# danini/multi-h

Measured on AMD Instinct MI355X. Metric: scored homography hypotheses/sec (50k pts x 100k models), higher is better.
Workload: dtype f64

## Files before the change

multi-h_amd/csrc/expand.hip:

```cpp

#include "mh_kernels.hpp"

#include <algorithm>
#include <atomic>
#include <chrono>

namespace mh {

enum { C_TLAST = 0,
       C_PEND = 1,
       C_ERROR = 2,
       C_ACCEPTED = 3,
       C_EXCESS_NODES = 4,
       C_ARRIVE = 5,
       C_TICKET = 6,
       C_FLOW_MOVES = 7,
       C_CORE = 8,
       C_MOVES_SOLVED = 16, C_CORE_MAX = 17, C_MOVES_RUN = 18, C_XCD_USED = 19,
       C_TOOK_N = 20,
       C_XCD = 64, C_LINE = 32, C_TOP = C_XCD + 8 * C_LINE,
       C_SUBTICKET = C_TOP + C_LINE, SUBTICKETS = 16,
       C_COUNT = EXPAND_FLAG_WORDS };
static_assert(C_SUBTICKET + SUBTICKETS * C_LINE <= C_COUNT, "control block too small");
constexpr int STRIPES = 64, STRIPE_LL = 16;
enum { A_DELTA_S = 64, A_ENERGY_S = A_DELTA_S + STRIPES * STRIPE_LL, A_EXCESS_S = A_ENERGY_S + STRIPES * STRIPE_LL,
       A_TOTAL = A_EXCESS_S + STRIPES * STRIPE_LL };
static_assert(A_TOTAL <= EXPAND_ACC_WORDS, "accumulator block too small");
enum { A_DELTA = 0, A_ENERGY = 1, A_EXCESS_SUM = 2, A_CORE_SUM = 3, A_OUTER = 4, A_RELAX = 5, A_PUSH = 6,
       A_BARRIERS = 7, A_TICKS = 8, A_T_BAR = 9, A_T_RELAX = 10, A_T_PUSH = 11, A_T_TAIL = 12, A_TAIL_ROUNDS = 13, A_MAX_WAIT = 14, A_COUNT = 16  };
enum { ERR_OVERFLOW = 1, ERR_BARRIER_TIMEOUT = 2, ERR_NO_CONVERGENCE = 3 };

struct MoveCtx {
    int* cap; int* sent; int* excess; int* sink_cap; int* height; int* decided; unsigned char* took; int* core;
    int* took_list;
    int* flags; long long* acc;
    int* saved_flow; int* saved_sink; int* trace; int* detail;
    int alpha, t, warm;
};
struct MoveBatch { MoveCtx c[EXPAND_MAX_CTX]; int count; };
enum { B_TLAST0 = 0,
       B_SEQ = 1,
       B_TICKET = 2,
       B_BAD = 8,
       B_WORDS = 8 + EXPAND_MAX_CTX };
static_assert(EXPAND_MAX_CTX <= 32, "one bit per move of a batch");
enum { HB_FIRST_INVALID = 0, HB_TLAST = 1, HB_ERROR = 2, HB_ACCEPTED_HERE = 3, HB_DIRTY = 4, HB_SEQ = 5, HB_WORDS = 8 };

#define LD(p) __hip_atomic_load((p), __ATOMIC_RELAXED, __HIP_MEMORY_SCOPE_AGENT)
#define ST(p, v) __hip_atomic_store((p), (v), __ATOMIC_RELAXED, __HIP_MEMORY_SCOPE_AGENT)

__device__ __forceinline__ bool move_is_skipped(const int* flags, int t, int L)
{
    return flags[C_ERROR] != 0 || (t >= L && flags[C_TLAST] <= t - L);
}

__global__ void k_ctl_init(MoveBatch b)
{
    int* flags = b.c[blockIdx.x].flags;
    long long* acc = b.c[blockIdx.x].acc;
    for (int t = threadIdx.x; t < C_COUNT; t += blockDim.x) flags[t] = (t == C_TLAST || t == C_PEND) ? -1 : 0;
    for (int t = threadIdx.x; t < A_TOTAL; t += blockDim.x) acc[t] = 0;
}

__global__ void __launch_bounds__(256)
k_init_labeling(const int* __restrict__ cost, int L, int n, const int* __restrict__ init,
                int* __restrict__ label, int* __restrict__ cur_cost)
{
    const int i = blockIdx.x * 256 + threadIdx.x;
    if (i >= n) return;
    const int l = init ? init[i] : 0;
    label[i] = l;
    cur_cost[i] = cost[(size_t)i * L + l];
}

__global__ void __launch_bounds__(256)
k_argmin_labels(const int* __restrict__ cost, int L, int n, int* __restrict__ label,
                long long* __restrict__ acc)
{
    const int i = blockIdx.x * 256 + threadIdx.x;
    long long mine = 0;
    if (i < n) {
        int best = 0, bc = cost[(size_t)i * L];
        for (int l = 1; l < L; ++l) {
            const int c = cost[(size_t)i * L + l];
            if (c < bc) { bc = c; best = l; }
        }
        label[i] = best;
        mine = bc;
    }
    __shared__ long long s[256];
    s[threadIdx.x] = mine;
    __syncthreads();
    for (int st = 128; st >= 1; st >>= 1) {
        if ((int)threadIdx.x < st) s[threadIdx.x] += s[threadIdx.x + st];
        __syncthreads();
    }
    if (threadIdx.x == 0)
        atomicAdd((unsigned long long*)&acc[A_ENERGY_S + (blockIdx.x % STRIPES) * STRIPE_LL], (unsigned long long)s[0]);
}

constexpr int LPN = 16;
constexpr int SITES_PER_BLOCK = 256 / LPN;

template <int CTRL>
__device__ __forceinline__ int dpp_mov(int v) { return __builtin_amdgcn_update_dpp(0, v, CTRL, 0xf, 0xf, true); }
template <int CTRL>
__device__ __forceinline__ long long dpp_mov64(long long v)
{
    const int lo = dpp_mov<CTRL>((int)(unsigned)((unsigned long long)v & 0xffffffffull)), hi = dpp_mov<CTRL>((int)(v >> 32));
    return (long long)(((unsigned long long)(unsigned)hi << 32) | (unsigned)lo);
}
constexpr int DPP_XOR1 = 0xB1, DPP_XOR2 = 0x4E, DPP_HALF_MIRROR = 0x141, DPP_MIRROR = 0x140;
template <int W>
__device__ __forceinline__ int row_min(int v)
{
    static_assert(W == 8 || W == 16, "a DPP row");
    int o = dpp_mov<DPP_XOR1>(v); v = o < v ? o : v;
    o = dpp_mov<DPP_XOR2>(v); v = o < v ? o : v;
    o = dpp_mov<DPP_HALF_MIRROR>(v); v = o < v ? o : v;
    if (W == 16) { o = dpp_mov<DPP_MIRROR>(v); v = o < v ? o : v; }
    return v;
}
template <int W>
__device__ __forceinline__ long long row_min64(long long v)
{
    static_assert(W == 8 || W == 16, "a DPP row");
    long long o = dpp_mov64<DPP_XOR1>(v); v = o < v ? o : v;
    o = dpp_mov64<DPP_XOR2>(v); v = o < v ? o : v;
    o = dpp_mov64<DPP_HALF_MIRROR>(v); v = o < v ? o : v;
    if (W == 16) { o = dpp_mov64<DPP_MIRROR>(v); v = o < v ? o : v; }
    return v;
}
template <int W>
__device__ __forceinline__ long long row_sum64(long long v)
{
    static_assert(W == 8 || W == 16, "a DPP row");
    v += dpp_mov64<DPP_XOR1>(v);
    v += dpp_mov64<DPP_XOR2>(v);
    v += dpp_mov64<DPP_HALF_MIRROR>(v);
    if (W == 16) v += dpp_mov64<DPP_MIRROR>(v);
    return v;
}
template <int W>
__device__ __forceinline__ int row_sum(int v)
{
    static_assert(W == 8 || W == 16, "a DPP row");
    v += dpp_mov<DPP_XOR1>(v);
    v += dpp_mov<DPP_XOR2>(v);
    v += dpp_mov<DPP_HALF_MIRROR>(v);
    if (W == 16) v += dpp_mov<DPP_MIRROR>(v);
    return v;
}

template <typename F>
__device__ __forceinline__ void for_flagged(unsigned long long mask, F body)
{
    const int grp = (int)(threadIdx.x & 63) / LPN;
    while (mask) {
        int b[4];
#pragma unroll
        for (int q = 0; q < 4; ++q) {
            b[q] = mask ? (int)__builtin_ctzll(mask) : -1;
            if (mask) mask &= mask - 1;
        }
        const int m = grp == 0 ? b[0] : grp == 1 ? b[1] : grp == 2 ? b[2] : b[3];
        body(m);
    }
}
constexpr int SPW = 16;
constexpr int SPW_MAX = 64;
constexpr int SITES_PER_WBLOCK_MAX = 4 * SPW_MAX;

__global__ void __launch_bounds__(256)
k_move_setup(Graph g, const int* __restrict__ cost, int L, int potts, int reduce_on,
             int* label, int* __restrict__ cur_cost, MoveBatch b, int spw)
{
    const MoveCtx& c = b.c[blockIdx.y];
    const int alpha = c.alpha, t = c.t;
    const unsigned char* __restrict__ took = c.took;
    int* __restrict__ cap = c.cap;
    int* __restrict__ excess = c.excess;
    int* __restrict__ sink_cap = c.sink_cap;
    int* __restrict__ decided = c.decided;
    int* __restrict__ flags = c.flags;
    long long* __restrict__ acc = c.acc;
    const int lane = threadIdx.x & 63;
    const int sub = threadIdx.x % LPN;
    const int s0 = (blockIdx.x * 4 + (int)(threadIdx.x >> 6)) * spw;
    const int i = s0 + lane;
    const bool in = lane < spw && i < g.n;
    const int pa = flags[C_PEND];
    int li = 0, cc = 0;
    if (in) {
        li = label[i];
        cc = cur_cost[i];
        if (pa >= 0 && took[i]) {
            li = pa;
            cc = cost[(size_t)i * L + pa];
            label[i] = pa; cur_cost[i] = cc;
        }
    }
    if (__shfl(move_is_skipped(flags, t, L) ? 1 : 0, 0)) return;
    long long K = 0;
    bool walk = false;
    if (in) {
        if (li == alpha) decided[i] = 3;
        else {
            K = cost[(size_t)i * L + alpha];
            if (reduce_on && K - cc > 2ll * potts * g.wsum[i]) decided[i] = 2;
            else walk = true;
        }
    }
    for_flagged(__ballot(walk), [&](int m) {
        const int mm = m < 0 ? 0 : m;
        const int li_m = __shfl(li, mm), cc_m = __shfl(cc, mm);
        const long long K_m = __shfl(K, mm);
        if (m < 0) return;
        const int im = s0 + m;
        const int k0 = g.rowptr[im], k1 = g.rowptr[im + 1];
        long long S = 0, out = 0, inn = 0;
        for (int k = k0 + sub; k < k1; k += LPN) {
            const int j = g.col[k];
            const long long wk64 = (long long)g.w[k] * potts;
            if (wk64 > 0x7fffffffll) atomicExch(&flags[C_ERROR], ERR_OVERFLOW);
            const int wk = wk64 > 0x7fffffffll ? 0x7fffffff : (int)wk64;
            int lj = label[j];
            if (pa >= 0 && took[j]) lj = pa;
            if (lj == alpha) { S += wk; cap[k] = 0; cap[g.rev[k]] = 0; }
            else if (j < im) { if (li_m != lj) S += wk; cap[k] = wk; out += wk; if (li_m == lj) inn += wk; }
            else { const int c = (li_m == lj) ? wk : 0; cap[k] = c; out += c; inn += wk; }
        }
        S = row_sum64<LPN>(S) + cc_m;
        out = row_sum64<LPN>(out);
        inn = row_sum64<LPN>(inn);
        if (sub != 0) return;
        const long long tr = S - K_m;
        if (tr > 0x7fffffffll || -tr > 0x7fffffffll) atomicExch(&flags[C_ERROR], ERR_OVERFLOW);
        const int ex = tr > 0 ? (int)tr : 0;
        excess[im] = ex;
        sink_cap[im] = tr < 0 ? (int)(-tr) : 0;
        int verdict = 0;
        if (reduce_on) {
            if (tr > out) verdict = 1;
            else if (-tr > inn) verdict = 2;
        }
        decided[im] = verdict;
        if (ex > 0) atomicAdd((unsigned long long*)&acc[A_EXCESS_S + (blockIdx.x % STRIPES) * STRIPE_LL], (unsigned long long)ex);
    });
}

template <bool COMPACT>
__global__ void __launch_bounds__(256)
k_reduce(Graph g, int L, MoveBatch b, int ROUNDS, int housekeep, int spw)
{
    const MoveCtx& c = b.c[blockIdx.y];
    const int t = c.t;
    int* cap = c.cap;
    int* excess = c.excess;
    int* sink_cap = c.sink_cap;
    int* decided = c.decided;
    int* __restrict__ flags = c.flags;
    long long* __restrict__ acc = c.acc;
    int* __restrict__ core = c.core;
    const int lane = threadIdx.x & 63;
    const int sub = threadIdx.x % LPN;
    const int slot = (blockIdx.x * 4 + (int)(threadIdx.x >> 6)) * spw + lane;
    const int u = (lane < spw && slot < g.n) ? (COMPACT ? g.order[slot] : slot) : -1;
    __shared__ int s_skip;
    __shared__ int s_cnt, s_base;
    __shared__ int s_list[SITES_PER_WBLOCK_MAX];
    if (threadIdx.x == 0) { s_skip = move_is_skipped(flags, t, L) ? 1 : 0; s_cnt = 0; }
    __syncthreads();
    const bool skipped = s_skip != 0;
    if (housekeep && blockIdx.x == 0 && threadIdx.x == 0) {
// ... 649 lines not shown
    __syncthreads();
    int rounds = 0;
    for (;;) {
        if (threadIdx.x == 0) s_changed = 0;
        __syncthreads();
        for (int i = threadIdx.x; i < g.n; i += 1024) {
            int c = comp[i];
            if (c < 0) continue;
            int m = c;
            for (int k = g.rowptr[i]; k < g.rowptr[i + 1]; ++k) { const int cj = comp[g.col[k]]; if (cj >= 0 && cj < m) m = cj; }
            if (m < c) { atomicMin(&comp[i], m); atomicMin(&comp[c], m); s_changed = 1; }
        }
        __syncthreads();
        for (int i = threadIdx.x; i < g.n; i += 1024) {
            int c = comp[i];
            if (c < 0) continue;
            while (comp[c] < c) c = comp[c];
            comp[i] = c;
        }
        __syncthreads();
        ++rounds;
        if (!s_changed || rounds > 4096) break;
        __syncthreads();
    }
    for (int i = threadIdx.x; i < g.n; i += 1024) if (comp[i] >= 0) { atomicAdd(&csize[comp[i]], 1); atomicAdd(&s_acc[0], 1); }
    __syncthreads();
    for (int i = threadIdx.x; i < g.n; i += 1024) {
        const int sz = csize[i];
        if (sz <= 0) continue;
        atomicAdd(&s_acc[1], 1);
        const int old = atomicMax(&s_acc[2], sz);
        atomicMax(&s_acc[3], old < sz ? old : sz);
        if (sz <= 64) { atomicAdd(&s_acc[4], sz); atomicAdd(&s_acc[9], 1); }
        if (sz <= 256) { atomicAdd(&s_acc[5], sz); atomicAdd(&s_acc[10], 1); }
        if (sz <= 1024) { atomicAdd(&s_acc[6], sz); atomicAdd(&s_acc[11], 1); }
        if (sz <= 2048) { atomicAdd(&s_acc[7], sz); atomicAdd(&s_acc[12], 1); }
        if (sz <= 8192) { atomicAdd(&s_acc[8], sz); atomicAdd(&s_acc[13], 1); }
    }
    __syncthreads();
    if (threadIdx.x < 16) out[threadIdx.x] = threadIdx.x == 14 ? rounds : s_acc[threadIdx.x];
}

__global__ void __launch_bounds__(SOLVE_THREADS)
k_solve(Graph g, int L, MoveBatch b, int mslots, SolveParams sp)
{
    const MoveCtx& c = b.c[blockIdx.y];
    const int t = c.t, warm = c.warm;
    int* cap = c.cap;
    int* sent = c.sent;
    int* excess = c.excess;
    int* sink_cap = c.sink_cap;
    int* height = c.height;
    int* decided = c.decided;
    const int* __restrict__ core = c.core;
    int* flags = c.flags;
    long long* acc = c.acc;
    int* __restrict__ trace = c.trace;
    int* __restrict__ detail = c.detail;
    int* __restrict__ saved_flow = c.saved_flow;
    int* __restrict__ saved_sink = c.saved_sink;
    extern __shared__ int s_priv[];
    __shared__ int s_red[8];
    __shared__ int s_skip;
    if (threadIdx.x == 0) s_skip = move_is_skipped(flags, t, L) ? 1 : 0;
    __syncthreads();
    if (s_skip) return;
    if (g.n >= H_MASK) { if (threadIdx.x == 0) atomicExch(&flags[C_ERROR], ERR_OVERFLOW); return; }
    int pre[EXPAND_CORE_SHARDS + 1];
    pre[0] = 0;
#pragma unroll
    for (int s = 0; s < EXPAND_CORE_SHARDS; ++s) pre[s + 1] = pre[s] + flags[C_CORE + s];
    const int K = pre[EXPAND_CORE_SHARDS];
    if (K == 0) return;
    int P = (K + SOLVE_ROWS - 1) / SOLVE_ROWS;
    if (P > (int)gridDim.x) P = (int)gridDim.x;
    if ((int)blockIdx.x >= P) return;
    if (K <= P * SOLVE_ROWS) solve_body<false>(g, t, cap, sent, excess, sink_cap, height, decided, core, flags, acc, trace, detail,
                                                saved_flow, saved_sink, warm, mslots, sp, s_priv, s_red, pre, K, P);
    else solve_body<true>(g, t, cap, sent, excess, sink_cap, height, decided, core, flags, acc, trace, detail,
                          saved_flow, saved_sink, warm, mslots, sp, s_priv, s_red, pre, K, P);
}

__global__ void __launch_bounds__(256)
k_delta(Graph g, const int* __restrict__ cost, int L, int potts,
        const int* __restrict__ label, const int* __restrict__ cur_cost, MoveBatch b, int spw)
{
    const MoveCtx& c = b.c[blockIdx.y];
    const int alpha = c.alpha, t = c.t;
    const int* __restrict__ decided = c.decided;
    unsigned char* __restrict__ took = c.took;
    int* __restrict__ flags = c.flags;
    long long* acc = c.acc;
    __shared__ long long s[256];
    __shared__ int s_last;
    if (threadIdx.x == 0) s_last = move_is_skipped(flags, t, L) ? 1 : 0;
    __syncthreads();
    if (s_last) return;
    const int lane = threadIdx.x & 63;
    const int sub = threadIdx.x % LPN;
    const int s0 = (blockIdx.x * 4 + (int)(threadIdx.x >> 6)) * spw;
    const int i = s0 + lane;
    long long mine = 0;
    int oi = 0;
    bool ti = false;
    if (lane < spw && i < g.n) {
        oi = label[i];
        ti = decided[i] == 1;
        took[i] = ti ? 1 : 0;
        if (ti) mine += (long long)cost[(size_t)i * L + alpha] - cur_cost[i];
    }
    if (c.took_list) {
        const unsigned long long tb = __ballot(ti);
        if (tb) {
            int base = 0;
            if (lane == 0) base = atomicAdd(&flags[C_TOOK_N], (int)__popcll(tb));
            base = __shfl(base, 0);
            if (ti) c.took_list[base + (int)__popcll(tb & ((1ull << lane) - 1ull))] = i;
        }
    }
    for_flagged(__ballot(ti), [&](int m) {
        const int oi_m = __shfl(oi, m < 0 ? 0 : m);
        if (m < 0) return;
        const int im = s0 + m;
        for (int k = g.rowptr[im] + sub; k < g.rowptr[im + 1]; k += LPN) {
            const int j = g.col[k];
            const bool tj = decided[j] == 1;
            if (tj && j > im) continue;
            const int oj = label[j];
            const int nj = tj ? alpha : oj;
            const int dn = (alpha != nj) - (oi_m != oj);
            mine += (long long)dn * g.w[k] * potts;
        }
    });
    s[threadIdx.x] = mine;
    __syncthreads();
    for (int st = 128; st >= 1; st >>= 1) {
        if ((int)threadIdx.x < st) s[threadIdx.x] += s[threadIdx.x + st];
        __syncthreads();
    }
    if (threadIdx.x == 0) {
        if (s[0] != 0) atomicAdd((unsigned long long*)&acc[A_DELTA_S + (blockIdx.x % STRIPES) * STRIPE_LL], (unsigned long long)s[0]);
        asm volatile("s_waitcnt vmcnt(0)" ::: "memory");
        const int st = (int)(blockIdx.x % SUBTICKETS);
        const int members = ((int)gridDim.x - st + SUBTICKETS - 1) / SUBTICKETS;
        int last = 0;
        if (atomicAdd(&flags[C_SUBTICKET + st * C_LINE], 1) == members - 1) {
            const int used = (int)gridDim.x < SUBTICKETS ? (int)gridDim.x : SUBTICKETS;
            last = atomicAdd(&flags[C_TICKET], 1) == used - 1;
        }
        s_last = last;
    }
    __syncthreads();
    if (s_last && threadIdx.x < 64) {
        long long d = (int)threadIdx.x < STRIPES ? LD(&acc[A_DELTA_S + threadIdx.x * STRIPE_LL]) : 0ll;
#pragma unroll
        for (int m = 32; m >= 1; m >>= 1) d += __shfl_xor(d, m, 64);
        if (threadIdx.x == 0 && d < 0) {
            flags[C_TLAST] = t;
            flags[C_PEND] = alpha;
            flags[C_ACCEPTED] += 1;
        }
        if (threadIdx.x == 0) {
            flags[C_MOVES_RUN] += 1;
            for (int s = 0; s < EXPAND_CORE_SHARDS; ++s) flags[C_CORE + s] = 0;
            for (int s = C_XCD; s < C_TOP + C_LINE; ++s) flags[s] = 0;
            flags[C_ARRIVE] = 0;
        }
    }
}

__global__ void __launch_bounds__(256)
k_apply_pending(int n, const int* __restrict__ cost, int L, int* __restrict__ label,
                int* __restrict__ cur_cost, const unsigned char* __restrict__ took,
                const int* __restrict__ flags, int )
{
    const int pa = flags[C_PEND];
    if (pa < 0) return;
    const int i = blockIdx.x * 256 + threadIdx.x;
    if (i < n && took[i]) {
        label[i] = pa;
        cur_cost[i] = cost[(size_t)i * L + pa];
    }
}



__global__ void k_batch_prep(MoveBatch b, int* __restrict__ bctl)
{
    int* G = b.c[0].flags;
    const int k = threadIdx.x;
    if (k == 0) { bctl[B_TLAST0] = G[C_TLAST]; G[C_PEND] = -1; }
    if (k < EXPAND_MAX_CTX) bctl[B_BAD + k] = 0;
    if (k >= 1 && k < b.count) {
        int* f = b.c[k].flags;
        f[C_TLAST] = G[C_TLAST];
        f[C_PEND] = -1;
        f[C_ERROR] = G[C_ERROR];
    }
}

__device__ __forceinline__ bool batch_move_skipped(const MoveCtx& c, int tlast0, int L)
{
    return c.flags[C_ERROR] != 0 || (c.t >= L && tlast0 <= c.t - L);
}

__global__ void __launch_bounds__(256)
k_batch_check(Graph g, const int* __restrict__ cost, int L, int potts, const int* __restrict__ label, const int* __restrict__ cur_cost,
              MoveBatch b, int* __restrict__ bctl)
{
    const int j = blockIdx.y;
    if (j + 1 >= b.count) return;
    const MoveCtx& cj = b.c[j];
    const int tlast0 = bctl[B_TLAST0];
    if (batch_move_skipped(cj, tlast0, L) || cj.flags[C_PEND] < 0) return;
    const int nt = cj.flags[C_TOOK_N];
    const int sub = threadIdx.x % LPN;
    const int alpha_j = cj.alpha, later = b.count - 1 - j;
    unsigned bad = 0;
    for (int idx = blockIdx.x * SITES_PER_BLOCK + (int)threadIdx.x / LPN; idx < nt; idx += gridDim.x * SITES_PER_BLOCK) {
        const int p = cj.took_list[idx];
        const int k0 = g.rowptr[p], k1 = g.rowptr[p + 1];
        for (int a = k0 + sub - (sub == 0 ? 1 : 0); a < k1; a = (a < k0 ? k0 : a + LPN)) {
            const int s_ = a < k0 ? p : g.col[a];
            const long long W = (long long)potts * g.wsum[s_];
            const int lb = label[s_];
            const long long Dl = cur_cost[s_];
            const int* row = cost + (size_t)s_ * L + (alpha_j + 1);
            const long long Dj = a < k0 ? (long long)cost[(size_t)s_ * L + alpha_j] : 0;
            for (int q = 0; q < later; ++q) {
                const long long Db = row[q];
                bool ok = lb == alpha_j + 1 + q || Db - Dl > W;
                if (ok && a < k0) ok = Db - Dj > W;
                if (!ok) bad |= 1u << (j + 1 + q);
            }
        }
    }
#pragma unroll
    for (int m = 32; m >= 1; m >>= 1) bad |= (unsigned)__shfl_xor((int)bad, m, 64);
    if ((threadIdx.x & 63) == 0 && bad) atomicOr((unsigned*)&bctl[B_BAD + j], bad);
}

struct CtxFlags { int* p[EXPAND_MAX_CTX]; };
__global__ void __launch_bounds__(256)
k_batch_commit(const int* __restrict__ cost, int L, int* __restrict__ label, int* __restrict__ cur_cost, MoveBatch b,
               int* __restrict__ bctl, int* __restrict__ h_batch, CtxFlags all_flags, int n_ctx_all)
{
    __shared__ int s_first, s_err, s_last_t, s_n_acc;
    __shared__ unsigned s_acc;
    __shared__ int s_ek[EXPAND_MAX_CTX], s_pend[EXPAND_MAX_CTX], s_nt[EXPAND_MAX_CTX];
    __shared__ unsigned s_bad[EXPAND_MAX_CTX];
    __shared__ int s_g[5];
    if ((int)threadIdx.x < b.count) {
        const int* f = b.c[threadIdx.x].flags;
        s_ek[threadIdx.x] = f[C_ERROR];
        s_pend[threadIdx.x] = f[C_PEND];
        s_nt[threadIdx.x] = f[C_TOOK_N];
        s_bad[threadIdx.x] = (unsigned)bctl[B_BAD + threadIdx.x];
    } else if (threadIdx.x >= 64 && threadIdx.x < 69) {
        const int q = threadIdx.x - 64;
        const int* G = b.c[0].flags;
        s_g[q] = q == 0 ? bctl[B_TLAST0] : q == 1 ? G[C_ERROR] : q == 2 ? G[C_TLAST] : q == 3 ? G[C_ACCEPTED] : bctl[B_SEQ];
    }
    __syncthreads();
    if (threadIdx.x == 0) {
        const int tlast0 = s_g[0];
        unsigned accepted = 0;
        int first_invalid = b.count, err = 0, last_t = -1, n_acc = 0;
        for (int k = 0; k < b.count; ++k) {
            const MoveCtx& c = b.c[k];
            const int ek = s_ek[k];
            const bool skipped = ek != 0 || (c.t >= L && tlast0 <= c.t - L);
            bool valid = true;
            if (accepted) {
                if (skipped) valid = false;
                else
                    for (int j = 0; j < k; ++j)
                        if ((accepted >> j & 1u) && (s_bad[j] >> k & 1u)) valid = false;
            }
            if (!valid) { first_invalid = k; break; }
            if (ek) err = ek;
            if (!skipped && s_pend[k] >= 0) { accepted |= 1u << k; last_t = c.t; ++n_acc; }
        }
        s_first = first_invalid; s_err = err; s_acc = accepted; s_last_t = last_t; s_n_acc = n_acc;
    }
    __syncthreads();
    const unsigned accepted = s_acc;
    for (int k = 0; k < b.count; ++k) {
        if (!(accepted >> k & 1u)) continue;
        const MoveCtx& c = b.c[k];
        const int nt = s_nt[k], a = c.alpha;
        for (int i = blockIdx.x * 256 + threadIdx.x; i < nt; i += gridDim.x * 256) {
            const int p = c.took_list[i];
            label[p] = a;
            cur_cost[p] = cost[(size_t)p * L + a];
        }
    }
    __shared__ int s_is_last;
    __syncthreads();
    if (threadIdx.x == 0) {
        __threadfence();
        s_is_last = atomicAdd(&bctl[B_TICKET], 1) == (int)gridDim.x - 1;
    }
    __syncthreads();
    if (s_is_last && threadIdx.x == 0) {
        bctl[B_TICKET] = 0;
        int* G = b.c[0].flags;
        const int g_err = s_g[1] ? s_g[1] : s_err;
        const int g_tlast = s_last_t > s_g[2] ? s_last_t : s_g[2];
        const int seq = s_g[4] + 1;
        if (g_err != s_g[1]) G[C_ERROR] = g_err;
        if (g_tlast != s_g[2]) G[C_TLAST] = g_tlast;
        G[C_ACCEPTED] = s_g[3] + s_n_acc - (int)(accepted & 1u);
        bctl[B_SEQ] = seq;
        h_batch[HB_FIRST_INVALID] = s_first;
        h_batch[HB_TLAST] = g_tlast;
        h_batch[HB_ERROR] = g_err;
        h_batch[HB_ACCEPTED_HERE] = s_n_acc;
        h_batch[HB_DIRTY] = 0;
        __threadfence_system();
        __hip_atomic_store(&h_batch[HB_SEQ], seq, __ATOMIC_RELEASE, __HIP_MEMORY_SCOPE_SYSTEM);
        bctl[B_TLAST0] = g_tlast;
        G[C_PEND] = -1;
        for (int k = 0; k < EXPAND_MAX_CTX; ++k) bctl[B_BAD + k] = 0;
        for (int k = 1; k < n_ctx_all; ++k) {
            int* f = all_flags.p[k];
            f[C_TLAST] = g_tlast;
            f[C_PEND] = -1;
            f[C_ERROR] = g_err;
        }
    }
}

__global__ void k_stats_merge(MoveBatch b)
{
    const int t = threadIdx.x;
    int* G = b.c[0].flags;
    long long* A = b.c[0].acc;
    const int fw[5] = { C_FLOW_MOVES, C_MOVES_SOLVED, C_MOVES_RUN, C_CORE_MAX, C_XCD_USED };
    if (t < 5) {
        const int w = fw[t];
        int v = G[w];
        for (int k = 1; k < b.count; ++k) {
            int* f = b.c[k].flags;
            if (t < 3) v += f[w]; else if (f[w] > v) v = f[w];
            f[w] = 0;
        }
        G[w] = v;
    } else if (t >= 8 && t - 8 + A_CORE_SUM < A_COUNT) {
        const int w = t - 8 + A_CORE_SUM;
        long long v = A[w];
        for (int k = 1; k < b.count; ++k) {
            long long* a = b.c[k].acc;
            if (w == A_MAX_WAIT) { if (a[w] > v) v = a[w]; } else v += a[w];
            a[w] = 0;
        }
        A[w] = v;
    }
}

__global__ void __launch_bounds__(256)
k_energy(Graph g, int potts, const int* __restrict__ label, const int* __restrict__ cur_cost,
         int* __restrict__ flags, long long* __restrict__ acc)
{
    if (blockIdx.x == 0 && threadIdx.x == 0) flags[C_PEND] = -1;
    const int i = blockIdx.x * SITES_PER_BLOCK + threadIdx.x / LPN;
    const int sub = threadIdx.x % LPN;
    long long mine = 0;
    if (i < g.n) {
        if (sub == 0) mine = cur_cost[i];
        const int li = label[i];
        for (int k = g.rowptr[i] + sub; k < g.rowptr[i + 1]; k += LPN) {
            const int j = g.col[k];
            if (j < i && label[j] != li) mine += (long long)g.w[k] * potts;
        }
    }
    __shared__ long long s[256];
    s[threadIdx.x] = mine;
    __syncthreads();
    for (int st = 128; st >= 1; st >>= 1) {
        if ((int)threadIdx.x < st) s[threadIdx.x] += s[threadIdx.x + st];
        __syncthreads();
    }
    if (threadIdx.x == 0)
        atomicAdd((unsigned long long*)&acc[A_ENERGY_S + (blockIdx.x % STRIPES) * STRIPE_LL], (unsigned long long)s[0]);
}

hipError_t launch_init_labeling(const int* cost, int L, int n, const int* init, int* label,
                                int* cur_cost, hipStream_t s)
{
    hipLaunchKernelGGL(k_init_labeling, dim3((n + 255) / 256), dim3(256), 0, s, cost, L, n, init,
                       label, cur_cost);
    return hipGetLastError();
}

hipError_t launch_argmin_labels(const int* cost, int L, int n, int* label, long long* acc,
                                hipStream_t s)
{
    hipLaunchKernelGGL(k_argmin_labels, dim3((n + 255) / 256), dim3(256), 0, s, cost, L, n, label,
                       acc);
    return hipGetLastError();
}

#define RET_IF(x) do { hipError_t e_ = (x); if (e_ != hipSuccess) return e_; } while (0)

__global__ void k_publish(const int* __restrict__ flags, long long* __restrict__ acc,
                          int* __restrict__ h_flags, long long* __restrict__ h_acc)
{
    const int t = threadIdx.x;
    if (t < EXPAND_HOST_WORDS) h_flags[t] = flags[t];
    long long en = t < STRIPES ? acc[A_ENERGY_S + t * STRIPE_LL] : 0ll;
    if (t < STRIPES) acc[A_ENERGY_S + t * STRIPE_LL] = 0;
#pragma unroll
    for (int m = 32; m >= 1; m >>= 1) en += __shfl_xor(en, m, 64);
    if (t < A_COUNT) h_acc[t] = t == A_ENERGY ? en : acc[t];
}

static hipError_t fetch(ExpandWork& w, ExpandStats& st, hipStream_t s)
{
    ++st.host_syncs;
    ++st.launches;
    hipLaunchKernelGGL(k_publish, dim3(1), dim3(64), 0, s, w.flags, w.acc, w.h_flags_dev, w.h_acc_dev);
    RET_IF(hipGetLastError());
    return hipStreamSynchronize(s);
}

hipError_t solver_blocks_per_cu(int* blocks)
{
    return hipOccupancyMaxActiveBlocksPerMultiprocessor(blocks, (const void*)k_solve, SOLVE_THREADS, sizeof(int) * F_FIELDS * SOLVE_ROWS);
}

hipError_t run_expansion(const Graph& g, const int* cost, int L, int potts, ExpandWork& w,
                         int max_cycles, ExpandStats* st, hipStream_t s)
{
    const dim3 grid1((g.n + 255) / 256), blk(256);
    const dim3 grid((g.n + SITES_PER_BLOCK - 1) / SITES_PER_BLOCK);
    auto spw_for = [&](int count) {
        if (w.batch_spw == 16 || w.batch_spw == 32 || w.batch_spw == 64) return w.batch_spw;
        const long long site_moves = (long long)count * g.n;
        return site_moves > (1ll << 19) ? 64 : site_moves > (1ll << 18) ? 32 : 16;
    };
    ExpandStats stats = {};
    const int n_ctx = std::max(1, std::min(w.n_ctx, EXPAND_MAX_CTX));
    MoveBatch all{};
    all.count = n_ctx;
    for (int k = 0; k < n_ctx; ++k) {
        MoveCtx& c = all.c[k];
        if (k == 0) { c.cap = w.cap; c.sent = w.sent; c.excess = w.excess; c.sink_cap = w.sink_cap; c.height = w.height; c.decided = w.decided;
                      c.took = w.took; c.core = w.core; c.flags = w.flags; c.acc = w.acc; c.took_list = w.took_list0; }
        else { const ExpandWork::Ctx& x = w.ctx[k - 1];
               c.cap = x.cap; c.sent = x.sent; c.excess = x.excess; c.sink_cap = x.sink_cap; c.height = x.height; c.decided = x.decided;
               c.took = x.took; c.core = x.core; c.flags = x.flags; c.acc = x.acc; c.took_list = x.took_list; }
    }
    hipLaunchKernelGGL(k_ctl_init, dim3(n_ctx), dim3(64), 0, s, all);
    RET_IF(hipGetLastError());
    ++stats.launches;
    auto finish_cycle = [&]() -> hipError_t {
        if (n_ctx > 1) { hipLaunchKernelGGL(k_stats_merge, dim3(1), dim3(64), 0, s, all); ++stats.launches; }
        return fetch(w, stats, s);
    };

    if (g.nnz == 0) {
        RET_IF(launch_argmin_labels(cost, L, g.n, w.label, w.acc, s));
        RET_IF(fetch(w, stats, s));
        stats.energy = w.h_acc[A_ENERGY];
        if (st) *st = stats;
        return hipSuccess;
    }

    long long energy = 0, old_energy = 0;
    hipLaunchKernelGGL(k_energy, grid, blk, 0, s, g, potts, w.label, w.cur_cost, w.flags, w.acc);
    RET_IF(fetch(w, stats, s));
    stats.launches += 1;
    energy = w.h_acc[A_ENERGY];
    if (energy > 0x7fffffffll) {
        stats.energy = -ERR_OVERFLOW;
        if (st) *st = stats;
        return hipErrorInvalidValue;
    }

    SolveParams sp{ w.reduce_rounds, w.relax_rounds, w.push_cycles, w.push_phases, w.push_mult > 0 ? w.push_mult : 1, 1 << 20, w.cascade_iters,
                    w.barrier_timeout_ticks > 0 ? (unsigned long long)w.barrier_timeout_ticks : 300000000ull,
                    w.barrier_first_timeout_ticks > 0 ? (unsigned long long)w.barrier_first_timeout_ticks : 300000000ull };
    int solve_grid = w.solve_grid > 0 ? w.solve_grid : 128;
    const int mslots = std::max(1, (g.n + solve_grid * SOLVE_ROWS - 1) / (solve_grid * SOLVE_ROWS));
    const size_t solve_lds = sizeof(int) * F_FIELDS * (size_t)mslots * SOLVE_ROWS;
    if (solve_lds > 128 * 1024) return hipErrorOutOfMemory;
    if (solve_lds > 48 * 1024)
        RET_IF(hipFuncSetAttribute((const void*)k_solve, hipFuncAttributeMaxDynamicSharedMemorySize, (int)solve_lds));

    CtxFlags all_flags{};
    for (int k = 0; k < n_ctx; ++k) all_flags.p[k] = all.c[k].flags;
    bool prepared = false;
    int group = 0;
    int injected_ctx = -1;
    auto enqueue_moves = [&](int alpha0, int t0, int count, int cycle) -> hipError_t {
        MoveBatch b = all;
        b.count = count;
        for (int k = 0; k < count; ++k) {
            MoveCtx& c = b.c[k];
            c.alpha = alpha0 + k;
            c.t = t0 + k;
            c.trace = (w.trace && c.t < w.trace_moves) ? w.trace : nullptr;
            c.detail = (w.trace && c.t == w.detail_move) ? w.trace + 8 * (size_t)w.trace_moves : nullptr;
            c.saved_flow = w.saved_flow ? w.saved_flow + (size_t)c.alpha * g.nnz : nullptr;
            c.saved_sink = w.saved_flow ? w.saved_sink + (size_t)c.alpha * g.n : nullptr;
            c.warm = (w.saved_flow && cycle > 1) ? 1 : 0;
            if (count == 1) c.took_list = nullptr;
        }
        const int spw = count > 1 ? spw_for(count) : SPW;
        const int spw_d = count > 1 ? SPW_MAX : SPW;
        const dim3 grid_w((unsigned)((g.n + 4 * spw - 1) / (4 * spw)), (unsigned)count);
        const dim3 grid_d((unsigned)((g.n + 4 * spw_d - 1) / (4 * spw_d)), (unsigned)count);
        if (count > 1 && !prepared) { hipLaunchKernelGGL(k_batch_prep, dim3(1), dim3(64), 0, s, b, w.bctl); ++stats.launches; }
        prepared = count > 1;
        hipLaunchKernelGGL(k_move_setup, grid_w, blk, 0, s, g, cost, L, potts, w.reduce_rounds > 0 ? 1 : 0, w.label, w.cur_cost, b, spw);
        if (w.reduce_launches > 1)
            hipLaunchKernelGGL(HIP_KERNEL_NAME(k_reduce<false>), grid_w, blk, 0, s, g, L, b, w.reduce_rounds, 1, spw);
        hipLaunchKernelGGL(HIP_KERNEL_NAME(k_reduce<true>), grid_w, blk, 0, s, g, L, b, w.reduce_rounds, w.reduce_launches > 1 ? 0 : 1, spw);
        if (count == 1 && w.comp_out && t0 < w.comp_moves)
            hipLaunchKernelGGL(k_core_components, dim3(1), dim3(1024), 0, s, g, L, t0, w.decided, w.flags, w.comp_scratch,
                               w.comp_scratch + g.n, w.comp_out + 16 * (size_t)t0);
        hipLaunchKernelGGL(k_solve, dim3((unsigned)solve_grid, (unsigned)count), dim3(SOLVE_THREADS), solve_lds, s, g, L, b, mslots, sp);
        injected_ctx = -1;
        if (++group == w.inject_group && w.inject_ctx < count) {
            RET_IF(hipMemsetD32Async((hipDeviceptr_t)(b.c[w.inject_ctx].flags + C_ERROR), ERR_NO_CONVERGENCE, 1, s));
            injected_ctx = w.inject_ctx;
        }
        hipLaunchKernelGGL(k_delta, grid_d, blk, 0, s, g, cost, L, potts, w.label, w.cur_cost, b, spw_d);
        if (count > 1) {
            hipLaunchKernelGGL(k_batch_check, dim3(32, (unsigned)count), blk, 0, s, g, cost, L, potts, w.label, w.cur_cost, b, w.bctl);
            hipLaunchKernelGGL(k_batch_commit, dim3(32), blk, 0, s, cost, L, w.label, w.cur_cost, b, w.bctl, w.h_batch_dev, all_flags, n_ctx);
            stats.launches += 2;
        }
        stats.launches += w.reduce_launches > 1 ? 5 : 4;
        if (w.reduce_rounds > 0) stats.reduce_launches += w.reduce_launches > 1 ? 2 : 1;
        return hipGetLastError();
    };

    const bool can_batch = n_ctx > 1 && w.bctl && w.h_batch && L >= 2 && !w.comp_out;
    bool batching = can_batch && L >= w.batch_min_labels;
    if (can_batch) {
        RET_IF(hipMemsetAsync(w.bctl, 0, sizeof(int) * B_WORDS, s));
        w.h_batch[HB_SEQ] = 0;
    }
    int host_tlast = -1;
    bool host_fresh = true;
    int bsize = n_ctx;
    int batch_seq = 0;
    int t = 0;
    for (int cycle = 1; cycle <= max_cycles; ++cycle) {
        old_energy = energy;
        int alpha = 0;
        if (can_batch && cycle >= 2) batching = true;
        while (alpha < L) {
            if (host_fresh && t >= L && host_tlast <= t - L) {
                const int rest = L - alpha;
                stats.moves += rest; stats.host_skipped += rest;
                alpha += rest; t += rest;
                break;
            }
            int B = std::min(bsize, L - alpha);
            if (host_fresh && t + B > host_tlast + L && host_tlast + L > t && t >= L) B = host_tlast + L - t;
            if (!batching || B < 2) {
                RET_IF(enqueue_moves(alpha, t, 1, cycle));
                ++stats.moves; ++stats.solo_moves;
                ++alpha; ++t;
                host_fresh = false;
                continue;
            }
            if (!host_fresh) {
                hipLaunchKernelGGL(k_apply_pending, grid1, blk, 0, s, g.n, cost, L, w.label, w.cur_cost, w.took, w.flags, 1);
                ++stats.launches;
            }
            RET_IF(enqueue_moves(alpha, t, B, cycle));
            ++stats.batches;
            ++stats.host_syncs;
            ++batch_seq;
            {
                volatile int* seq_word = w.h_batch + HB_SEQ;
                const auto t_poll = std::chrono::steady_clock::now();
                bool seen = false;
                for (int spin = 0;; ++spin) {
                    if (*seq_word == batch_seq) { seen = true; break; }
                    if ((spin & 255) == 255 && std::chrono::steady_clock::now() - t_poll > std::chrono::milliseconds(2)) break;
                }
                if (seen) std::atomic_thread_fence(std::memory_order_acquire);
                else RET_IF(hipStreamSynchronize(s));
                if (w.h_batch[HB_SEQ] != batch_seq) return hipErrorUnknown;
            }
            if (w.h_batch[HB_ERROR]) break;
            const int j = w.h_batch[HB_FIRST_INVALID];
            if (injected_ctx >= j) ++stats.injected_discarded;
            host_tlast = w.h_batch[HB_TLAST];
            host_fresh = true;
            stats.moves += j; stats.batch_committed += j;
            alpha += j; t += j;
            if (j < B) {
                ++stats.batch_invalid;
                if (2 * j < B) bsize = std::max(2, bsize / 2);
            } else if (B == bsize) bsize = std::min(n_ctx, 2 * bsize);
        }
        hipLaunchKernelGGL(k_apply_pending, grid1, blk, 0, s, g.n, cost, L, w.label, w.cur_cost, w.took, w.flags, 0);
        hipLaunchKernelGGL(k_energy, grid, blk, 0, s, g, potts, w.label, w.cur_cost, w.flags, w.acc);
        stats.launches += 2;
        RET_IF(finish_cycle());
        stats.cycles = cycle;
        if (w.h_flags[C_ERROR]) {
            stats.energy = -(long long)w.h_flags[C_ERROR];
            if (st) *st = stats;
            return w.h_flags[C_ERROR] == ERR_OVERFLOW ? hipErrorInvalidValue : hipErrorLaunchTimeOut;
        }
        host_tlast = w.h_flags[C_TLAST];
        host_fresh = true;
        energy = w.h_acc[A_ENERGY];
        if (energy == old_energy) break;
    }
    stats.energy = energy;
    stats.accepted = w.h_flags[C_ACCEPTED];
    stats.flow_moves = w.h_flags[C_FLOW_MOVES];
    stats.moves_solved = w.h_flags[C_MOVES_SOLVED];
    stats.moves_run = w.h_flags[C_MOVES_RUN];
    stats.core_sites = w.h_acc[A_CORE_SUM];
    stats.core_max = w.h_flags[C_CORE_MAX];
    stats.outer_iterations = w.h_acc[A_OUTER];
    stats.relax_intervals = w.h_acc[A_RELAX];
// ... 15 lines not shown
```

Measured before the change: 13.41 million.

## Fuse delta, batch check and commit into one move-tail kernel

Merges the separate k_delta, k_batch_check and k_batch_commit kernels (and removes k_batch_prep) into a single k_move_tail kernel. It computes the batch-conflict bits inline while walking each taken site's neighbourhood, then elects a last block via tickets to commit accepted moves and reset per-context flags. bctl initialisation moves into k_ctl_init. The aim is to cut per-batch kernel launches and the redundant second pass over took_list and neighbours, at the price of the commit running serially in one block and more complex ticket synchronisation.

```diff
diff --git a/multi-h_amd/csrc/expand.hip b/multi-h_amd/csrc/expand.hip
--- a/multi-h_amd/csrc/expand.hip
+++ b/multi-h_amd/csrc/expand.hip
@@ -54,10 +54,12 @@
     return flags[C_ERROR] != 0 || (t >= L && flags[C_TLAST] <= t - L);
 }
 
-__global__ void k_ctl_init(MoveBatch b)
+__global__ void k_ctl_init(MoveBatch b, int* __restrict__ bctl)
 {
     int* flags = b.c[blockIdx.x].flags;
     long long* acc = b.c[blockIdx.x].acc;
+    if (blockIdx.x == 0 && bctl)
+        for (int t = threadIdx.x; t < B_WORDS; t += blockDim.x) bctl[t] = t == B_TLAST0 ? -1 : 0;
     for (int t = threadIdx.x; t < C_COUNT; t += blockDim.x) flags[t] = (t == C_TLAST || t == C_PEND) ? -1 : 0;
     for (int t = threadIdx.x; t < A_TOTAL; t += blockDim.x) acc[t] = 0;
 }
@@ -189,7 +191,7 @@
     const int s0 = (blockIdx.x * 4 + (int)(threadIdx.x >> 6)) * spw;
     const int i = s0 + lane;
     const bool in = lane < spw && i < g.n;
-    const int pa = flags[C_PEND];
+    const int pa = b.count > 1 ? -1 : flags[C_PEND];
     int li = 0, cc = 0;
     if (in) {
         li = label[i];
@@ -1005,64 +1007,109 @@
 }
 
 __global__ void __launch_bounds__(256)
-k_delta(Graph g, const int* __restrict__ cost, int L, int potts,
-        const int* __restrict__ label, const int* __restrict__ cur_cost, MoveBatch b, int spw)
-{
-    const MoveCtx& c = b.c[blockIdx.y];
+k_apply_pending(int n, const int* __restrict__ cost, int L, int* __restrict__ label,
+                int* __restrict__ cur_cost, const unsigned char* __restrict__ took,
+                const int* __restrict__ flags, int )
+{
+    const int pa = flags[C_PEND];
+    if (pa < 0) return;
+    const int i = blockIdx.x * 256 + threadIdx.x;
+    if (i < n && took[i]) {
+        label[i] = pa;
+        cur_cost[i] = cost[(size_t)i * L + pa];
+    }
+}
+
+
+
+struct CtxFlags { int* p[EXPAND_MAX_CTX]; };
+__global__ void __launch_bounds__(256)
+k_move_tail(Graph g, const int* __restrict__ cost, int L, int potts, int* label, int* cur_cost, MoveBatch b, int spw,
+            int* bctl, int* h_batch, CtxFlags all_flags, int n_ctx_all)
+{
+    const int y = blockIdx.y;
+    const MoveCtx& c = b.c[y];
     const int alpha = c.alpha, t = c.t;
     const int* __restrict__ decided = c.decided;
     unsigned char* __restrict__ took = c.took;
-    int* __restrict__ flags = c.flags;
+    int* flags = c.flags;
     long long* acc = c.acc;
     __shared__ long long s[256];
-    __shared__ int s_last;
-    if (threadIdx.x == 0) s_last = move_is_skipped(flags, t, L) ? 1 : 0;
-    __syncthreads();
-    if (s_last) return;
-    const int lane = threadIdx.x & 63;
-    const int sub = threadIdx.x % LPN;
-    const int s0 = (blockIdx.x * 4 + (int)(threadIdx.x >> 6)) * spw;
-    const int i = s0 + lane;
-    long long mine = 0;
-    int oi = 0;
-    bool ti = false;
-    if (lane < spw && i < g.n) {
-        oi = label[i];
-        ti = decided[i] == 1;
-        took[i] = ti ? 1 : 0;
-        if (ti) mine += (long long)cost[(size_t)i * L + alpha] - cur_cost[i];
-    }
-    if (c.took_list) {
-        const unsigned long long tb = __ballot(ti);
-        if (tb) {
-            int base = 0;
-            if (lane == 0) base = atomicAdd(&flags[C_TOOK_N], (int)__popcll(tb));
-            base = __shfl(base, 0);
-            if (ti) c.took_list[base + (int)__popcll(tb & ((1ull << lane) - 1ull))] = i;
-        }
-    }
-    for_flagged(__ballot(ti), [&](int m) {
-        const int oi_m = __shfl(oi, m < 0 ? 0 : m);
-        if (m < 0) return;
-        const int im = s0 + m;
-        for (int k = g.rowptr[im] + sub; k < g.rowptr[im + 1]; k += LPN) {
-            const int j = g.col[k];
-            const bool tj = decided[j] == 1;
-            if (tj && j > im) continue;
-            const int oj = label[j];
-            const int nj = tj ? alpha : oj;
-            const int dn = (alpha != nj) - (oi_m != oj);
-            mine += (long long)dn * g.w[k] * potts;
-        }
-    });
-    s[threadIdx.x] = mine;
-    __syncthreads();
-    for (int st = 128; st >= 1; st >>= 1) {
-        if ((int)threadIdx.x < st) s[threadIdx.x] += s[threadIdx.x + st];
+    __shared__ int s_flag;
+    if (threadIdx.x == 0) s_flag = move_is_skipped(flags, t, L) ? 1 : 0;
+    __syncthreads();
+    const bool skipped = s_flag != 0;
+    __syncthreads();
+    if (!skipped) {
+        const int lane = threadIdx.x & 63;
+        const int sub = threadIdx.x % LPN;
+        const int s0 = (blockIdx.x * 4 + (int)(threadIdx.x >> 6)) * spw;
+        const int i = s0 + lane;
+        const int later = b.count - 1 - y;
+        long long mine = 0;
+        unsigned bad = 0;
+        int oi = 0;
+        bool ti = false;
+        if (lane < spw && i < g.n) {
+            oi = label[i];
+            ti = decided[i] == 1;
+            took[i] = ti ? 1 : 0;
+            if (ti) mine += (long long)cost[(size_t)i * L + alpha] - cur_cost[i];
+        }
+        if (c.took_list) {
+            const unsigned long long tb = __ballot(ti);
+            if (tb) {
+                int base = 0;
+                if (lane == 0) base = atomicAdd(&flags[C_TOOK_N], (int)__popcll(tb));
+                base = __shfl(base, 0);
+                if (ti) ST(&c.took_list[base + (int)__popcll(tb & ((1ull << lane) - 1ull))], i);
+            }
+        }
+        for_flagged(__ballot(ti), [&](int m) {
+            const int oi_m = __shfl(oi, m < 0 ? 0 : m);
+            if (m < 0) return;
+            const int im = s0 + m;
+            const int k0 = g.rowptr[im], k1 = g.rowptr[im + 1];
+            for (int k = k0 + sub; k < k1; k += LPN) {
+                const int j = g.col[k];
+                const bool tj = decided[j] == 1;
+                if (tj && j > im) continue;
+                const int oj = label[j];
+                const int nj = tj ? alpha : oj;
+                const int dn = (alpha != nj) - (oi_m != oj);
+                mine += (long long)dn * g.w[k] * potts;
+            }
+            if (later <= 0) return;
+            for (int a = k0 + sub - (sub == 0 ? 1 : 0); a < k1; a = (a < k0 ? k0 : a + LPN)) {
+                const int s_ = a < k0 ? im : g.col[a];
+                const long long W = (long long)potts * g.wsum[s_];
+                const int lb = label[s_];
+                const long long Dl = cur_cost[s_];
+                const int* row = cost + (size_t)s_ * L + (alpha + 1);
+                const long long Dj = a < k0 ? (long long)cost[(size_t)s_ * L + alpha] : 0;
+                for (int q = 0; q < later; ++q) {
+                    const long long Db = row[q];
+                    bool ok = lb == alpha + 1 + q || Db - Dl > W;
+                    if (ok && a < k0) ok = Db - Dj > W;
+                    if (!ok) bad |= 1u << (y + 1 + q);
+                }
+            }
+        });
+        if (later > 0) {
+#pragma unroll
+            for (int m = 32; m >= 1; m >>= 1) bad |= (unsigned)__shfl_xor((int)bad, m, 64);
+            if (lane == 0 && bad) atomicOr((unsigned*)&bctl[B_BAD + y], bad);
+        }
+        asm volatile("s_waitcnt vmcnt(0)" ::: "memory");
+        s[threadIdx.x] = mine;
         __syncthreads();
+        for (int st = 128; st >= 1; st >>= 1) {
+            if ((int)threadIdx.x < st) s[threadIdx.x] += s[threadIdx.x + st];
+            __syncthreads();
+        }
     }
     if (threadIdx.x == 0) {
-        if (s[0] != 0) atomicAdd((unsigned long long*)&acc[A_DELTA_S + (blockIdx.x % STRIPES) * STRIPE_LL], (unsigned long long)s[0]);
+        if (!skipped && s[0] != 0) atomicAdd((unsigned long long*)&acc[A_DELTA_S + (blockIdx.x % STRIPES) * STRIPE_LL], (unsigned long long)s[0]);
         asm volatile("s_waitcnt vmcnt(0)" ::: "memory");
         const int st = (int)(blockIdx.x % SUBTICKETS);
         const int members = ((int)gridDim.x - st + SUBTICKETS - 1) / SUBTICKETS;
@@ -1071,118 +1118,62 @@
             const int used = (int)gridDim.x < SUBTICKETS ? (int)gridDim.x : SUBTICKETS;
             last = atomicAdd(&flags[C_TICKET], 1) == used - 1;
         }
-        s_last = last;
-    }
-    __syncthreads();
-    if (s_last && threadIdx.x < 64) {
+        s_flag = last;
+    }
+    __syncthreads();
+    if (!s_flag) return;
+
+    if (!skipped && threadIdx.x < 64) {
         long long d = (int)threadIdx.x < STRIPES ? LD(&acc[A_DELTA_S + threadIdx.x * STRIPE_LL]) : 0ll;
 #pragma unroll
         for (int m = 32; m >= 1; m >>= 1) d += __shfl_xor(d, m, 64);
-        if (threadIdx.x == 0 && d < 0) {
-            flags[C_TLAST] = t;
-            flags[C_PEND] = alpha;
-            flags[C_ACCEPTED] += 1;
-        }
         if (threadIdx.x == 0) {
+            if (d < 0) {
+                ST(&flags[C_TLAST], t);
+                ST(&flags[C_PEND], alpha);
+                ST(&flags[C_ACCEPTED], flags[C_ACCEPTED] + 1);
+            }
             flags[C_MOVES_RUN] += 1;
-            for (int s = 0; s < EXPAND_CORE_SHARDS; ++s) flags[C_CORE + s] = 0;
-            for (int s = C_XCD; s < C_TOP + C_LINE; ++s) flags[s] = 0;
+            for (int q = 0; q < EXPAND_CORE_SHARDS; ++q) flags[C_CORE + q] = 0;
+            for (int q = C_XCD; q < C_TOP + C_LINE; ++q) flags[q] = 0;
             flags[C_ARRIVE] = 0;
         }
     }
-}
-
-__global__ void __launch_bounds__(256)
-k_apply_pending(int n, const int* __restrict__ cost, int L, int* __restrict__ label,
-                int* __restrict__ cur_cost, const unsigned char* __restrict__ took,
-                const int* __restrict__ flags, int )
-{
-    const int pa = flags[C_PEND];
-    if (pa < 0) return;
-    const int i = blockIdx.x * 256 + threadIdx.x;
-    if (i < n && took[i]) {
-        label[i] = pa;
-        cur_cost[i] = cost[(size_t)i * L + pa];
-    }
-}
-
-
-
-__global__ void k_batch_prep(MoveBatch b, int* __restrict__ bctl)
-{
-    int* G = b.c[0].flags;
-    const int k = threadIdx.x;
-    if (k == 0) { bctl[B_TLAST0] = G[C_TLAST]; G[C_PEND] = -1; }
-    if (k < EXPAND_MAX_CTX) bctl[B_BAD + k] = 0;
-    if (k >= 1 && k < b.count) {
-        int* f = b.c[k].flags;
-        f[C_TLAST] = G[C_TLAST];
-        f[C_PEND] = -1;
-        f[C_ERROR] = G[C_ERROR];
-    }
-}
-
-__device__ __forceinline__ bool batch_move_skipped(const MoveCtx& c, int tlast0, int L)
-{
-    return c.flags[C_ERROR] != 0 || (c.t >= L && tlast0 <= c.t - L);
-}
-
-__global__ void __launch_bounds__(256)
-k_batch_check(Graph g, const int* __restrict__ cost, int L, int potts, const int* __restrict__ label, const int* __restrict__ cur_cost,
-              MoveBatch b, int* __restrict__ bctl)
-{
-    const int j = blockIdx.y;
-    if (j + 1 >= b.count) return;
-    const MoveCtx& cj = b.c[j];
-    const int tlast0 = bctl[B_TLAST0];
-    if (batch_move_skipped(cj, tlast0, L) || cj.flags[C_PEND] < 0) return;
-    const int nt = cj.flags[C_TOOK_N];
-    const int sub = threadIdx.x % LPN;
-    const int alpha_j = cj.alpha, later = b.count - 1 - j;
-    unsigned bad = 0;
-    for (int idx = blockIdx.x * SITES_PER_BLOCK + (int)threadIdx.x / LPN; idx < nt; idx += gridDim.x * SITES_PER_BLOCK) {
-        const int p = cj.took_list[idx];
-        const int k0 = g.rowptr[p], k1 = g.rowptr[p + 1];
-        for (int a = k0 + sub - (sub == 0 ? 1 : 0); a < k1; a = (a < k0 ? k0 : a + LPN)) {
-            const int s_ = a < k0 ? p : g.col[a];
-            const long long W = (long long)potts * g.wsum[s_];
-            const int lb = label[s_];
-            const long long Dl = cur_cost[s_];
-            const int* row = cost + (size_t)s_ * L + (alpha_j + 1);
-            const long long Dj = a < k0 ? (long long)cost[(size_t)s_ * L + alpha_j] : 0;
-            for (int q = 0; q < later; ++q) {
-                const long long Db = row[q];
-                bool ok = lb == alpha_j + 1 + q || Db - Dl > W;
-                if (ok && a < k0) ok = Db - Dj > W;
-                if (!ok) bad |= 1u << (j + 1 + q);
-            }
-        }
-    }
-#pragma unroll
-    for (int m = 32; m >= 1; m >>= 1) bad |= (unsigned)__shfl_xor((int)bad, m, 64);
-    if ((threadIdx.x & 63) == 0 && bad) atomicOr((unsigned*)&bctl[B_BAD + j], bad);
-}
-
-struct CtxFlags { int* p[EXPAND_MAX_CTX]; };
-__global__ void __launch_bounds__(256)
-k_batch_commit(const int* __restrict__ cost, int L, int* __restrict__ label, int* __restrict__ cur_cost, MoveBatch b,
-               int* __restrict__ bctl, int* __restrict__ h_batch, CtxFlags all_flags, int n_ctx_all)
-{
+    if (!h_batch) {
+        if (threadIdx.x == 0 && bctl) {
+            const int g_tlast = LD(&flags[C_TLAST]), g_err = LD(&flags[C_ERROR]);
+            bctl[B_TLAST0] = g_tlast;
+            for (int k = 1; k < n_ctx_all; ++k) {
+                int* f = all_flags.p[k];
+                f[C_TLAST] = g_tlast;
+                f[C_PEND] = -1;
+                f[C_ERROR] = g_err;
+            }
+        }
+        return;
+    }
+    if (threadIdx.x == 0) {
+        asm volatile("s_waitcnt vmcnt(0)" ::: "memory");
+        s_flag = atomicAdd(&bctl[B_TICKET], 1) == (int)gridDim.y - 1;
+    }
+    __syncthreads();
+    if (!s_flag) return;
+
     __shared__ int s_first, s_err, s_last_t, s_n_acc;
     __shared__ unsigned s_acc;
     __shared__ int s_ek[EXPAND_MAX_CTX], s_pend[EXPAND_MAX_CTX], s_nt[EXPAND_MAX_CTX];
     __shared__ unsigned s_bad[EXPAND_MAX_CTX];
     __shared__ int s_g[5];
     if ((int)threadIdx.x < b.count) {
-        const int* f = b.c[threadIdx.x].flags;
-        s_ek[threadIdx.x] = f[C_ERROR];
-        s_pend[threadIdx.x] = f[C_PEND];
-        s_nt[threadIdx.x] = f[C_TOOK_N];
-        s_bad[threadIdx.x] = (unsigned)bctl[B_BAD + threadIdx.x];
+        int* f = b.c[threadIdx.x].flags;
+        s_ek[threadIdx.x] = LD(&f[C_ERROR]);
+        s_pend[threadIdx.x] = LD(&f[C_PEND]);
+        s_nt[threadIdx.x] = LD(&f[C_TOOK_N]);
+        s_bad[threadIdx.x] = (unsigned)LD(&bctl[B_BAD + threadIdx.x]);
     } else if (threadIdx.x >= 64 && threadIdx.x < 69) {
         const int q = threadIdx.x - 64;
-        const int* G = b.c[0].flags;
-        s_g[q] = q == 0 ? bctl[B_TLAST0] : q == 1 ? G[C_ERROR] : q == 2 ? G[C_TLAST] : q == 3 ? G[C_ACCEPTED] : bctl[B_SEQ];
+        int* G = b.c[0].flags;
+        s_g[q] = LD(q == 0 ? &bctl[B_TLAST0] : q == 1 ? &G[C_ERROR] : q == 2 ? &G[C_TLAST] : q == 3 ? &G[C_ACCEPTED] : &bctl[B_SEQ]);
     }
     __syncthreads();
     if (threadIdx.x == 0) {
@@ -1190,55 +1181,34 @@
         unsigned accepted = 0;
         int first_invalid = b.count, err = 0, last_t = -1, n_acc = 0;
         for (int k = 0; k < b.count; ++k) {
-            const MoveCtx& c = b.c[k];
+            const MoveCtx& ck = b.c[k];
             const int ek = s_ek[k];
-            const bool skipped = ek != 0 || (c.t >= L && tlast0 <= c.t - L);
+            const bool skipped_k = ek != 0 || (ck.t >= L && tlast0 <= ck.t - L);
             bool valid = true;
             if (accepted) {
-                if (skipped) valid = false;
+                if (skipped_k) valid = false;
                 else
                     for (int j = 0; j < k; ++j)
                         if ((accepted >> j & 1u) && (s_bad[j] >> k & 1u)) valid = false;
             }
             if (!valid) { first_invalid = k; break; }
             if (ek) err = ek;
-            if (!skipped && s_pend[k] >= 0) { accepted |= 1u << k; last_t = c.t; ++n_acc; }
+            if (!skipped_k && s_pend[k] >= 0) { accepted |= 1u << k; last_t = ck.t; ++n_acc; }
         }
         s_first = first_invalid; s_err = err; s_acc = accepted; s_last_t = last_t; s_n_acc = n_acc;
-    }
-    __syncthreads();
-    const unsigned accepted = s_acc;
-    for (int k = 0; k < b.count; ++k) {
-        if (!(accepted >> k & 1u)) continue;
-        const MoveCtx& c = b.c[k];
-        const int nt = s_nt[k], a = c.alpha;
-        for (int i = blockIdx.x * 256 + threadIdx.x; i < nt; i += gridDim.x * 256) {
-            const int p = c.took_list[i];
-            label[p] = a;
-            cur_cost[p] = cost[(size_t)p * L + a];
-        }
-    }
-    __shared__ int s_is_last;
-    __syncthreads();
-    if (threadIdx.x == 0) {
-        __threadfence();
-        s_is_last = atomicAdd(&bctl[B_TICKET], 1) == (int)gridDim.x - 1;
-    }
-    __syncthreads();
-    if (s_is_last && threadIdx.x == 0) {
         bctl[B_TICKET] = 0;
         int* G = b.c[0].flags;
-        const int g_err = s_g[1] ? s_g[1] : s_err;
-        const int g_tlast = s_last_t > s_g[2] ? s_last_t : s_g[2];
+        const int g_err = s_g[1] ? s_g[1] : err;
+        const int g_tlast = last_t > s_g[2] ? last_t : s_g[2];
         const int seq = s_g[4] + 1;
         if (g_err != s_g[1]) G[C_ERROR] = g_err;
         if (g_tlast != s_g[2]) G[C_TLAST] = g_tlast;
-        G[C_ACCEPTED] = s_g[3] + s_n_acc - (int)(accepted & 1u);
+        G[C_ACCEPTED] = s_g[3] + n_acc - (int)(accepted & 1u);
         bctl[B_SEQ] = seq;
-        h_batch[HB_FIRST_INVALID] = s_first;
+        h_batch[HB_FIRST_INVALID] = first_invalid;
         h_batch[HB_TLAST] = g_tlast;
         h_batch[HB_ERROR] = g_err;
-        h_batch[HB_ACCEPTED_HERE] = s_n_acc;
+        h_batch[HB_ACCEPTED_HERE] = n_acc;
         h_batch[HB_DIRTY] = 0;
         __threadfence_system();
         __hip_atomic_store(&h_batch[HB_SEQ], seq, __ATOMIC_RELEASE, __HIP_MEMORY_SCOPE_SYSTEM);
@@ -1250,6 +1220,23 @@
             f[C_TLAST] = g_tlast;
             f[C_PEND] = -1;
             f[C_ERROR] = g_err;
+        }
+    }
+    __syncthreads();
+    const unsigned accepted = s_acc;
+    for (int k = 0; k < b.count; ++k) {
+        if (!(accepted >> k & 1u)) continue;
+        const MoveCtx& ck = b.c[k];
+        const int nt = s_nt[k], a = ck.alpha;
+        for (int i0 = threadIdx.x; i0 < nt; i0 += 4 * 256) {
+            int p[4], cc[4];
+#pragma unroll
+            for (int q = 0; q < 4; ++q) p[q] = i0 + q * 256 < nt ? LD(&ck.took_list[i0 + q * 256]) : -1;
+#pragma unroll
+            for (int q = 0; q < 4; ++q) cc[q] = p[q] >= 0 ? cost[(size_t)p[q] * L + a] : 0;
+#pragma unroll
+            for (int q = 0; q < 4; ++q)
+                if (p[q] >= 0) { label[p[q]] = a; cur_cost[p[q]] = cc[q]; }
         }
     }
 }
@@ -1374,7 +1361,7 @@
                c.cap = x.cap; c.sent = x.sent; c.excess = x.excess; c.sink_cap = x.sink_cap; c.height = x.height; c.decided = x.decided;
                c.took = x.took; c.core = x.core; c.flags = x.flags; c.acc = x.acc; c.took_list = x.took_list; }
     }
-    hipLaunchKernelGGL(k_ctl_init, dim3(n_ctx), dim3(64), 0, s, all);
+    hipLaunchKernelGGL(k_ctl_init, dim3(n_ctx), dim3(64), 0, s, all, w.bctl);
     RET_IF(hipGetLastError());
     ++stats.launches;
     auto finish_cycle = [&]() -> hipError_t {
@@ -1411,9 +1398,9 @@
     if (solve_lds > 48 * 1024)
         RET_IF(hipFuncSetAttribute((const void*)k_solve, hipFuncAttributeMaxDynamicSharedMemorySize, (int)solve_lds));
 
+    const bool can_batch = n_ctx > 1 && w.bctl && w.h_batch && L >= 2 && !w.comp_out;
     CtxFlags all_flags{};
     for (int k = 0; k < n_ctx; ++k) all_flags.p[k] = all.c[k].flags;
-    bool prepared = false;
     int group = 0;
     int injected_ctx = -1;
     auto enqueue_moves = [&](int alpha0, int t0, int count, int cycle) -> hipError_t {
@@ -1434,8 +1421,6 @@
         const int spw_d = count > 1 ? SPW_MAX : SPW;
         const dim3 grid_w((unsigned)((g.n + 4 * spw - 1) / (4 * spw)), (unsigned)count);
         const dim3 grid_d((unsigned)((g.n + 4 * spw_d - 1) / (4 * spw_d)), (unsigned)count);
-        if (count > 1 && !prepared) { hipLaunchKernelGGL(k_batch_prep, dim3(1), dim3(64), 0, s, b, w.bctl); ++stats.launches; }
-        prepared = count > 1;
         hipLaunchKernelGGL(k_move_setup, grid_w, blk, 0, s, g, cost, L, potts, w.reduce_rounds > 0 ? 1 : 0, w.label, w.cur_cost, b, spw);
         if (w.reduce_launches > 1)
             hipLaunchKernelGGL(HIP_KERNEL_NAME(k_reduce<false>), grid_w, blk, 0, s, g, L, b, w.reduce_rounds, 1, spw);
@@ -1449,21 +1434,15 @@
             RET_IF(hipMemsetD32Async((hipDeviceptr_t)(b.c[w.inject_ctx].flags + C_ERROR), ERR_NO_CONVERGENCE, 1, s));
             injected_ctx = w.inject_ctx;
         }
-        hipLaunchKernelGGL(k_delta, grid_d, blk, 0, s, g, cost, L, potts, w.label, w.cur_cost, b, spw_d);
-        if (count > 1) {
-            hipLaunchKernelGGL(k_batch_check, dim3(32, (unsigned)count), blk, 0, s, g, cost, L, potts, w.label, w.cur_cost, b, w.bctl);
-            hipLaunchKernelGGL(k_batch_commit, dim3(32), blk, 0, s, cost, L, w.label, w.cur_cost, b, w.bctl, w.h_batch_dev, all_flags, n_ctx);
-            stats.launches += 2;
-        }
+        hipLaunchKernelGGL(k_move_tail, grid_d, blk, 0, s, g, cost, L, potts, w.label, w.cur_cost, b, spw_d, can_batch ? w.bctl : nullptr,
+                           count > 1 ? w.h_batch_dev : nullptr, all_flags, n_ctx);
         stats.launches += w.reduce_launches > 1 ? 5 : 4;
         if (w.reduce_rounds > 0) stats.reduce_launches += w.reduce_launches > 1 ? 2 : 1;
         return hipGetLastError();
     };
 
-    const bool can_batch = n_ctx > 1 && w.bctl && w.h_batch && L >= 2 && !w.comp_out;
     bool batching = can_batch && L >= w.batch_min_labels;
     if (can_batch) {
-        RET_IF(hipMemsetAsync(w.bctl, 0, sizeof(int) * B_WORDS, s));
         w.h_batch[HB_SEQ] = 0;
     }
     int host_tlast = -1;
```

Result: no change. 13.41 million, median of 2 (+0.0%).
